# genometools/vstree

Measured on AMD Instinct MI355X. Metric: queries/sec (100 bp queries, vmatch -mum -l 20 semantics, 3 Gbp ESA index resident in HBM), higher is better.
Workload: dtype u8; 1 GPU; 3 Gbp synthetic DNA index, 10 M x 100 bp queries per GPU, -mum -l 20; index_bp=3000000000, queries_per_gpu=10000000, query_len=100, minlen=20, prefixlength=13, index_bytes_hbm=115012207262, reads_in_hbm=two bits per symbol, 32 bytes per read (vsa_pack_reads), parallelism=index replicated, queries sharded x1

## Files before the change

### vstree_amd/csrc/esa_search.hip

```cpp
#include "search_host.hpp"
#include <rocprim/rocprim.hpp>
#include <type_traits>

#include "search_complete.inc"
#include "search_query.inc"
#include "mum_workplan.inc"
#include "mem_workplan.inc"
#include "mum_filter.inc"
#include "candidate_sort.inc"
#include <atomic>


namespace
{


enum class Form
{
  Ref,
  Deep,
  Staged,
  Rows,
  Windows
};
// ... 370 lines not shown
        cand.as<vsa_match>(), ncand, lenbits, k1.as<uint64_t>(),
        i1.as<uint32_t>());
    VSA_HIP(hipGetLastError());
    if (sort_radix<uint32_t>(k1.as<uint64_t>(), i1.as<uint32_t>(), s, 0,
                             lenbits + dbbits, stream) ||
        mumfilter_tiles<true>(
            s, s.pairs(lenbits, GatheredRecord{cand.as<vsa_match>()}), carry,
            stream, mums, &c))
    {
      return -100;
    }
  }
  *nmums = c.nmums;
  *sumlength = c.sumlength;
  return 0;
}

struct RecordForm
{
  bool keeppairs;
  bool packed;
  unsigned int lenbits, dbbits;
  uint32_t packbits, valbits;
  size_t recsize;
};

int recordform(const vsa_index *index, const vsa_queries *queries, bool domum,
               bool domumcand, bool ordered, uint32_t forcebits,
               RecordForm *rf)
{
  const unsigned int need = bitsfor(queries->maxlength);
  rf->keeppairs = domum && domumcand && !ordered && forcebits != 0;
  rf->lenbits = rf->keeppairs ? forcebits : need;
  rf->dbbits = bitsfor(index->n);
  rf->packed = domum && (!domumcand || rf->keeppairs) &&
               rf->lenbits + rf->dbbits <= 64 && rf->lenbits >= need &&
               queries->maxlength < 0xFFFFu &&
               ((queries->nq + queries->seqoffset) >> 48) == 0;
  if (rf->keeppairs && !rf->packed)
  {
    VSA_ERROR("packed candidates: %u length bits do not fit this batch "
              "(longest query %lu, index %lu)", forcebits,
              (unsigned long) queries->maxlength, (unsigned long) index->n);
    return -2;
  }
  rf->packbits = rf->packed ? rf->lenbits : 0;
  const bool small = ((queries->nq << rf->lenbits) >> 32) == 0;
  rf->valbits = (rf->packed && !rf->keeppairs && small) ? rf->lenbits : 0;
  rf->recsize = rf->valbits != 0 ? 4 : (rf->packed ? 8 : sizeof(vsa_match));
  return 0;
}

int compact_into(const RecordForm &form, DevBuf &raw, DevBuf &rawkeys,
                 uint64_t cap, DevBuf &cursors, DevBuf &doff, DevBuf &out,
                 DevBuf &keys, uint64_t at, hipStream_t stream)
{
  auto launch = [&](auto rec) {
    using REC = decltype(rec);
    k_compact_shards<REC><<<VSA_CURSOR_SHARDS, VSA_BLOCK, 0, stream>>>(
        raw.as<REC>(), rawkeys.as<uint64_t>(), cap,
        cursors.as<unsigned long long>(), doff.as<uint64_t>(),
        out.as<REC>() + at, keys.as<uint64_t>() + at);
  };
  if (form.valbits != 0)
  {
    launch(uint32_t());
  } else if (form.packed)
  {
    launch(uint64_t());
  } else
  {
    launch(vsa_match());
  }
  VSA_HIP(hipGetLastError());
  return 0;
}

struct QueryRun
{
  const vsa_index *index;
  const vsa_queries *queries;
  hipStream_t stream;
  DevQueries qs;
  bool domum, domumcand, ordered;
  uint32_t searchlength;
  RecordForm rec;
  Timer tall, tsearch, tfirst;
  DevBuf base;
  const uint64_t *dbase = nullptr;
  uint32_t perquery = 0;
  uint64_t nitems = 0;
  bool reduce = false, memplan = false;
  Form form = Form::Ref;
  DevBuf wcount, wtemp, wplan, wlist, wfirste, wfmlen, wfmdb, wboffset;
  const uint64_t *nlistword = nullptr;
  DevBuf pcursor, pdoff, psummary, prawout, prawkeys;
  uint64_t pcap = 0;
  bool fromplan = false, planemit = false;
  uint64_t plansearches = 0;
  DevBuf cursor, doff, summary, blocksum, rtemp, rawout, rawkeys, out, keys;
  uint64_t shardcap = 0, needed = 0, nplan = 0, nfirst = 0, plannedwork = 0;
  uint64_t plannedlocates = 0;
  double searchms = 0;

  QueryRun(const vsa_index *ix, const vsa_queries *q, bool mum, bool cand,
           bool ord, uint32_t least)
      : index(ix), queries(q), stream(ix->stream), qs(devqueries(q)),
        domum(mum), domumcand(cand), ordered(ord), searchlength(least),
        tall(stream), tsearch(stream), tfirst(stream)
  {
  }
};

template <typename IDX>
int workitems(QueryRun &st)
{
  const uint64_t nqr = st.queries->nq, least = st.searchlength;
  if (st.qs.uniformlen != 0)
  {
    st.perquery = (st.qs.uniformlen >= least) ? st.qs.uniformlen - least + 1
                                              : 0;
    st.nitems = (uint64_t) st.perquery * nqr;
    return 0;
  }
  DevBuf btemp;
  auto items = rocprim::make_transform_iterator(
      rocprim::counting_iterator<uint64_t>(0),
      [len = st.qs.length, nqr, least] __device__(uint64_t q) -> uint64_t {
        if (q >= nqr)
        {
          return 0;
        }
        const uint64_t l = len[q];
        return l >= least ? l - least + 1 : 0;
      });
  if (st.base.alloc((nqr + 1) * 8))
  {
    return -100;
  }
  VSA_HIP(rocprim_run(btemp, [&](void *p, size_t &tb) {
    return rocprim::exclusive_scan(p, tb, items, st.base.as<uint64_t>(),
                                   (uint64_t) 0, (size_t) (nqr + 1),
                                   rocprim::plus<uint64_t>(), st.stream);
  }));
  st.dbase = st.base.as<uint64_t>();
  const Fetch f = {st.dbase + nqr, 8};
  return fetchwords(st.stream, &f, 1, &st.nitems) ? -100 : 0;
}

int decide(QueryRun &st)
{
  const vsa_index *index = st.index;
  const vsa_queries *queries = st.queries;
  const uint64_t maxoffsets =
      (queries->maxlength >= st.searchlength)
          ? queries->maxlength - st.searchlength + 1
          : 0;
  if (st.domum && queries->maxlength >= 255 && index->lcpquirk < 0)
  {
    uint8_t b = 0;
    if (index->n >= 2)
    {
      VSA_HIP(hipMemcpyAsync(&b, index->lcp + index->n - 1, 1,
                             hipMemcpyDeviceToHost, st.stream));
      VSA_HIP(hipStreamSynchronize(st.stream));
    }
    index->lcpquirk = (b == 255) ? 1 : 0;
  }
  const bool exhaustive = (index->tune & 2u) != 0;
  const bool planable = maxoffsets > 1 && maxoffsets < 0xFFFFu &&
                        queries->nq < 0xFFFFFFFFull && !exhaustive;
  st.reduce = st.domum && planable &&
              !(queries->maxlength >= 255 && index->lcpquirk != 0);
  st.memplan = !st.domum && planable && index->esa8 != nullptr &&
               st.searchlength >= index->D && st.searchlength <= 255;
  st.form = pickform(index, queries, st.qs,
                     st.reduce ? Stage::MumFirst : Stage::Bytes,
                     st.searchlength);
  if (queries->rows != nullptr && st.form < Form::Rows)
  {
    if (vsa_queries_bytes(queries, st.stream) != 0)
    {
      return -100;
    }
    st.qs = devqueries(queries);
  }
  return 0;
}

template <typename IDX>
int first_pass(QueryRun &st, const DevIndex<IDX> &ix, Form form,
               uint64_t *blockcount)
{
  st.tfirst.start();
  withform(form, [&](auto deep, auto pq, auto rows, auto windows) {
    k_mum_first<IDX, deep, pq, rows, windows>
        <<<gridfor(st.queries->nq), VSA_BLOCK, ldsbytes(form, st.qs),
           st.stream>>>(ix, st.qs, st.perquery, st.searchlength,
                        st.wcount.as<uint32_t>(), st.wfirste.as<uint32_t>(),
                        st.wfmlen.as<uint32_t>(), st.wfmdb.as<uint64_t>(),
                        blockcount);
  });
  st.tfirst.stop();
  VSA_HIP(hipGetLastError());
  return 0;
}

int alloc_first(QueryRun &st)
{
  const uint64_t nq = st.queries->nq;
  return st.wcount.alloc((nq + 1) * 4) || st.wfirste.alloc(nq * 4) ||
         st.wfmlen.alloc(nq * 4) || st.wfmdb.alloc(nq * 8) ||
         st.wplan.alloc(nq * sizeof(PlanRanges));
}

int plan_emit(QueryRun &st, uint32_t rounds, PlanEmit *em)
{
  const uint32_t nshards = VSA_CURSOR_SHARDS;
  const uint64_t nb = blocksfor(st.queries->nq),
                 pershard = (nb + nshards - 1) / nshards;
  st.pcap = pershard * VSA_BLOCK * rounds;
  if (st.pcursor.alloc((size_t) nshards * VSA_CURSOR_STRIDE * 8) ||
      st.pdoff.alloc(nshards * 8) || st.psummary.alloc(4 * 8) ||
      st.prawout.alloc(nshards * st.pcap * st.rec.recsize) ||
      st.prawkeys.alloc(nshards * st.pcap * 8))
  {
    return -100;
  }
  VSA_HIP(hipMemsetAsync(st.pcursor.p, 0,
                         (size_t) nshards * VSA_CURSOR_STRIDE * 8, st.stream));
  em->base = st.dbase;
  em->perquery = st.perquery;
  em->out = st.prawout.as<vsa_match>();
  em->outkey = st.prawkeys.as<uint64_t>();
  em->shardcap = st.pcap;
  em->shardmask = nshards - 1;
  em->cursors = st.pcursor.as<unsigned long long>();
  em->packbits = st.rec.packbits;
  em->valbits = st.rec.valbits;
  st.planemit = true;
  return 0;
}

hipError_t plan_summary(QueryRun &st)
{
  return shard_summary(st.pcursor.as<unsigned long long>(), VSA_CURSOR_SHARDS,
                       st.pdoff.as<uint64_t>(), st.psummary.as<uint64_t>(),
                       st.stream);
}

template <typename IDX>
int mem_plan(QueryRun &st, const DevIndex<IDX> &ix)
{
  const vsa_index *index = st.index;
  const uint64_t nq = st.queries->nq;
  if (index->repbits == nullptr || index->repleast != st.searchlength)
  {
    if (index->repbits == nullptr)
    {
      VSA_HIP(vsa_hip_malloc((void **) &index->repbits,
                             ((index->n + 1) / 32 + 4) * 4));
    }
    VSA_HIP(hipMemsetAsync(index->repbits, 0, ((index->n + 1) / 32 + 4) * 4,
                           st.stream));
    k_repeat_bits<IDX><<<vsa_grid(blocksfor((index->n + 16) / 16)),
                         VSA_BLOCK, 0, st.stream>>>(
        ix.lcp, ix.suf, index->n, st.searchlength, index->repbits);
    VSA_HIP(hipGetLastError());
    index->repleast = st.searchlength;
  }
  const Form first = pickform(index, st.queries, st.qs, Stage::MemFirst,
                              st.searchlength);
  PlanEmit em;
  if (alloc_first(st) || first_pass(st, ix, first, nullptr) ||
      plan_emit(st, VSA_PLAN_ROUNDS, &em))
  {
    return -100;
  }
  k_mem_plan<IDX><<<gridfor(nq), VSA_BLOCK, 0, st.stream>>>(
      ix, st.qs, st.perquery, st.searchlength, st.wfirste.as<uint32_t>(),
      st.wfmdb.as<uint64_t>(), index->repbits, st.wcount.as<uint32_t>(),
      st.wplan.as<PlanRanges>(), em);
  VSA_HIP(hipGetLastError());
  VSA_HIP(plan_summary(st));
  st.fromplan = true;
  st.plansearches = nq;
  return 0;
}

int dump_planfile(QueryRun &st, const char *pf)
{
  const uint64_t k = std::min<uint64_t>(st.queries->nq, 65536);
  std::vector<uint32_t> hc(k), hp(k * VSA_PLAN_RANGES);
  VSA_HIP(hipMemcpyAsync(hc.data(), st.wcount.p, k * 4,
                         hipMemcpyDeviceToHost, st.stream));
  VSA_HIP(hipMemcpyAsync(hp.data(), st.wplan.p, k * sizeof(PlanRanges),
                         hipMemcpyDeviceToHost, st.stream));
  VSA_HIP(hipStreamSynchronize(st.stream));
  if (FILE *f = fopen(pf, "wb"))
  {
    for (uint64_t q = 0; q < k; q++)
    {
      (void) fwrite(&hc[q], 4, 1, f);
      (void) fwrite(&hp[q * VSA_PLAN_RANGES], 4, VSA_PLAN_RANGES, f);
    }
    fclose(f);
  }
  return 0;
}

template <typename IDX>
int mum_plan(QueryRun &st, const DevIndex<IDX> &ix)
{
  const uint64_t nq = st.queries->nq;
  if (alloc_first(st) || st.wlist.alloc(nq * 4))
  {
    return -100;
  }
  VSA_HIP(hipMemsetAsync(st.wcount.as<uint32_t>() + nq, 0, 4, st.stream));
  const uint64_t nb = blocksfor(nq), nbr = vsa_grid_blocks(nb);
  DevBuf bcount;
  if (bcount.alloc((nbr + 1) * 8) || st.wboffset.alloc((nbr + 1) * 8))
  {
    return -100;
  }
  VSA_HIP(hipMemsetAsync(bcount.as<uint64_t>() + nb, 0, 8, st.stream));
  if (first_pass(st, ix, st.form, bcount.as<uint64_t>()))
  {
    return -100;
  }
  VSA_HIP(rocprim_run(st.wtemp, [&](void *p, size_t &tb) {
    return rocprim::exclusive_scan(p, tb, bcount.as<uint64_t>(),
                                   st.wboffset.as<uint64_t>(), (uint64_t) 0,
                                   (size_t) (nb + 1), rocprim::plus<uint64_t>(),
                                   st.stream);
  }));
  k_wanted_fill<<<vsa_grid(nb), VSA_BLOCK, 0, st.stream>>>(
      st.wcount.as<uint32_t>(), nq, 0u, st.wboffset.as<uint64_t>(),
      st.wlist.as<uint32_t>());
  VSA_HIP(hipGetLastError());
  st.nlistword = st.wboffset.as<uint64_t>() + nb;
  PlanEmit em = PlanEmit();
  if (st.form != Form::Ref && plan_emit(st, VSA_PLAN_ROUNDS - 1, &em))
  {
    return -100;
  }
  withform(st.form, [&](auto deep, auto, auto rows, auto) {
    k_mum_plan<IDX, deep, deep, rows><<<gridfor(nq), VSA_BLOCK, 0, st.stream>>>(
        ix, st.qs, st.wlist.as<uint32_t>(), st.nlistword, st.searchlength,
        st.wfirste.as<uint32_t>(), st.wcount.as<uint32_t>(),
        st.wplan.as<PlanRanges>(), em);
  });
  if (st.planemit)
  {
    VSA_HIP(plan_summary(st));
  }
  VSA_HIP(hipGetLastError());
  const char *pf = getenv("VSA_DEBUG_PLANFILE");
  if (pf != nullptr && dump_planfile(st, pf))
  {
    return -100;
  }
  st.fromplan = true;
  return 0;
}

bool tilequeue(const QueryRun &st)
{
  return st.fromplan && st.domum && (st.index->tune & 32u) == 0;
}

template <typename IDX>
int walkgrid(const QueryRun &st, uint32_t *grid)
{
  const vsa_index *index = st.index;
  if (index->walkgridasked != 0)
  {
    *grid = index->walkgridasked;
    return 0;
  }
  hipError_t e = hipSuccess;
  withform(st.form, [&](auto deep, auto, auto rows, auto) {
    uint32_t &kept = index->walkgrid[deep ? 1 : 0][rows ? 1 : 0];
    if (kept == 0)
    {
      int percu = 0, cus = 0;
      e = hipOccupancyMaxActiveBlocksPerMultiprocessor(
          &percu, k_mum_walk_tiles<IDX, deep, rows>, 256, 0);
      if (e == hipSuccess)
      {
        e = hipDeviceGetAttribute(&cus, hipDeviceAttributeMultiprocessorCount,
                                  index->device);
      }
      if (e == hipSuccess)
      {
        kept = (uint32_t) std::max(percu, 1) * (uint32_t) std::max(cus, 1);
      }
    }
    *grid = kept;
  });
  VSA_HIP(e);
  return 0;
}

template <typename IDX>
void launch_search(QueryRun &st, const DevIndex<IDX> &ix,
                   uint64_t nplanblocks, uint32_t regions)
{
  withform(st.form, [&](auto deep, auto, auto rows, auto) {
    auto tiles = [&]() {
      unsigned long long *cursors = st.cursor.as<unsigned long long>();
      k_mum_walk_tiles<IDX, deep, rows>
          <<<vsa_grid(nplanblocks), 256, 0, st.stream>>>(
              ix, st.qs, st.dbase, st.perquery, st.wplan.as<PlanRanges>(),
              st.wcount.as<uint32_t>(), st.wlist.as<uint32_t>(), st.nlistword,
              cursors + (size_t) VSA_CURSOR_SHARDS * VSA_CURSOR_STRIDE,
              st.searchlength, st.rawout.as<vsa_match>(),
              st.rawkeys.as<uint64_t>(), st.shardcap, regions - 1, cursors,
              st.rec.packbits, st.rec.valbits,
              st.blocksum.as<PlannedWork>(), st.index->walkshift);
    };
    auto planned = [&](auto mum) {
      k_query_search_planned<IDX, 256, deep, rows, mum>
          <<<vsa_grid(nplanblocks), 256, 0, st.stream>>>(
              ix, st.qs, st.dbase, st.perquery, st.wplan.as<PlanRanges>(),
              st.wcount.as<uint32_t>(), st.searchlength,
              st.rawout.as<vsa_match>(), st.rawkeys.as<uint64_t>(),
              st.shardcap, VSA_CURSOR_SHARDS - 1,
              st.cursor.as<unsigned long long>(), st.rec.packbits,
              st.rec.valbits, st.blocksum.as<PlannedWork>(),
              st.index->walkshift);
    };
    auto unplanned = [&](auto mum) {
      k_query_search<IDX, mum, deep, 256>
          <<<vsa_grid((st.nitems + 255) / 256), 256, 0, st.stream>>>(
              ix, st.qs, st.dbase, st.perquery, st.nitems, st.searchlength,
              st.rawout.as<vsa_match>(), st.rawkeys.as<uint64_t>(),
              st.shardcap, VSA_CURSOR_SHARDS - 1,
              st.cursor.as<unsigned long long>(), st.rec.packbits,
              st.rec.valbits);
    };
    if (tilequeue(st))
    {
      tiles();
    } else if (st.fromplan && st.domum)
    {
      planned(std::true_type());
    } else if (st.fromplan)
    {
      if constexpr (deep && !rows)
      {
        planned(std::false_type());
      }
    } else if (st.nitems > 0 && st.domum)
    {
      unplanned(std::true_type());
    } else if (st.nitems > 0)
    {
      unplanned(std::false_type());
    }
  });
}

template <typename IDX>
int search(QueryRun &st, const DevIndex<IDX> &ix)
{
  const uint32_t nshards = VSA_CURSOR_SHARDS;
  const uint64_t perblock = 256 * (st.domum ? VSA_WALK_READS : 1);
  uint64_t nplanblocks = (st.queries->nq + perblock - 1) / perblock;
  uint64_t persum = 1;
  size_t rbytes = 0;
  if (tilequeue(st))
  {
    uint32_t grid = 0;
    if (walkgrid<IDX>(st, &grid))
    {
      return -100;
    }
    nplanblocks = grid;
    persum = 4;
  }
  const uint64_t nsums = persum * nplanblocks;
  if (st.fromplan)
  {
    if (st.blocksum.alloc((persum * vsa_grid_blocks(nplanblocks) + 1) *
                          sizeof(PlannedWork)))
    {
      return -100;
    }
    VSA_HIP(rocprim::reduce(nullptr, rbytes, st.blocksum.as<PlannedWork>(),
                            (PlannedWork *) nullptr, PlannedWork{0, 0},
                            (size_t) nsums, PlannedWorkPlus(), st.stream));
    if (st.rtemp.alloc(rbytes))
    {
      return -100;
    }
  }
  const size_t cursorbytes = (size_t) (nshards + 1) * VSA_CURSOR_STRIDE * 8;
  if (st.cursor.alloc(cursorbytes) || st.doff.alloc(nshards * 8) ||
      st.summary.alloc(6 * 8))
  {
    return -100;
  }
  st.shardcap =
      std::max<uint64_t>((st.queries->nq * 2 / nshards) * 5 / 4 + 64, 256);
  uint64_t maxshard = 0;
  uint32_t regions = nshards;
  for (int attempt = 0; attempt < 2; attempt++)
  {
    if (st.rawout.alloc(regions * st.shardcap * st.rec.recsize) ||
        st.rawkeys.alloc(regions * st.shardcap * 8))
    {
      return -100;
    }
    VSA_HIP(hipMemsetAsync(st.cursor.p, 0, cursorbytes, st.stream));
    st.tsearch.start();
    launch_search(st, ix, nplanblocks, regions);
    st.tsearch.stop();
    VSA_HIP(hipGetLastError());
    if (st.fromplan)
    {
      VSA_HIP(rocprim::reduce(
          st.rtemp.p, rbytes, st.blocksum.as<PlannedWork>(),
          reinterpret_cast<PlannedWork *>(st.summary.as<uint64_t>() + 4),
          PlannedWork{0, 0}, (size_t) nsums, PlannedWorkPlus(), st.stream));
    }
    const uint64_t *sm = st.summary.as<uint64_t>();
    VSA_HIP(shard_summary(st.cursor.as<unsigned long long>(), nshards,
                          st.doff.as<uint64_t>(), st.summary.as<uint64_t>(),
                          st.stream));
    const Fetch f[8] = {{sm, 8}, {sm + 1, 8}, {sm + 2, 8}, {sm + 3, 8},
                        {sm + 4, 8}, {st.planemit ? st.psummary.p : sm, 8},
                        {st.nlistword != nullptr ? st.nlistword : sm, 8},
                        {sm + 5, 8}};
    uint64_t got[8];
    if (fetchwords(st.stream, f, 8, got))
    {
      return -100;
    }
    if (st.nlistword != nullptr)
    {
      st.nfirst = got[6] >> 32;
      st.plansearches = 2 * (got[6] & 0xFFFFFFFFull);
    }
    st.nplan = st.planemit ? got[5] : 0;
    st.needed = got[0];
    maxshard = got[1];
    st.plannedlocates = st.fromplan ? got[4] : 0;
    st.plannedwork = st.fromplan ? got[7] : 0;
    st.searchms += st.tsearch.ms();
    if (maxshard <= st.shardcap)
    {
      return 0;
    }
    st.shardcap = maxshard;
    if (tilequeue(st))
    {
      regions = 1;
      st.shardcap = st.needed;
    }
  }
  VSA_ERROR("match buffer overflow: %llu > %llu",
            (unsigned long long) maxshard, (unsigned long long) st.shardcap);
  return -5;
}

int compact(QueryRun &st)
{
  const uint64_t total = st.needed + st.nplan + st.nfirst;
  if (total == 0)
  {
    return 0;
  }
  if (st.out.alloc(total * st.rec.recsize) || st.keys.alloc(total * 8) ||
      (st.nplan > 0 &&
       compact_into(st.rec, st.prawout, st.prawkeys, st.pcap, st.pcursor,
                    st.pdoff, st.out, st.keys, st.needed, st.stream)) ||
      (st.needed > 0 &&
       compact_into(st.rec, st.rawout, st.rawkeys, st.shardcap, st.cursor,
                    st.doff, st.out, st.keys, 0, st.stream)))
  {
    return -100;
  }
  if (st.nfirst > 0)
  {
    k_append_first<<<gridfor(st.queries->nq), VSA_BLOCK, 0, st.stream>>>(
        st.wfmlen.as<uint32_t>(), st.wfmdb.as<uint64_t>(),
        st.wboffset.as<uint64_t>(), st.queries->nq, st.perquery, st.dbase,
        st.qs.seqoffset, st.needed + st.nplan, st.out.as<vsa_match>(),
        st.keys.as<uint64_t>(), st.rec.packbits, st.rec.valbits);
    VSA_HIP(hipGetLastError());
  }
  st.needed = total;
  return 0;
}

#define VSA_CS_MINPAIRS (1u << 14)

std::atomic<uint64_t> g_cs_runs{0}, g_cs_overflows{0}, g_cs_longruns{0},
    g_cs_shift{0}, g_cs_buckets{0};

bool feedsbuckets(const QueryRun &st)
{
  const uint64_t total = st.needed + st.nplan + st.nfirst;
  const uint32_t tune = st.index->tune;
  if (!(st.domum && !st.domumcand && st.rec.packed && (tune & 4u) == 0 &&
        total > 0 && (total >= VSA_CS_MINPAIRS || (tune & 8u) != 0) &&
        cs_geometry(st.index->n, total, st.rec.lenbits, st.rec.dbbits)
                .nbuckets <= VSA_CS_MAXBUCKETS))
  {
    return false;
  }
  if ((tune & 8u) == 0 && st.index->cs_skip > 0)
  {
    st.index->cs_skip--;
    return false;
  }
  return true;
}

template <typename VAL>
int mumfilter_buckets(QueryRun &st, DevBuf &mums, MumCounts *c)
{
  const RecordForm &rec = st.rec;
  const uint64_t total = st.needed + st.nplan + st.nfirst;
  CsSources src = CsSources();
  if (st.needed > 0)
  {
    src.reg[0] = {st.rawout.p, st.rawkeys.as<uint64_t>(),
                  st.cursor.as<unsigned long long>(), st.shardcap, st.needed};
  }
  if (st.nplan > 0)
  {
    src.reg[1] = {st.prawout.p, st.prawkeys.as<uint64_t>(),
                  st.pcursor.as<unsigned long long>(), st.pcap, st.nplan};
  }
  if (st.nfirst > 0)
  {
    src.first = {st.wfmlen.as<uint32_t>(), st.wfmdb.as<uint64_t>(),
                 st.queries->nq, st.qs.seqoffset, rec.packbits, rec.valbits};
  }
  CsGeometry g;
  if (mums.alloc(total * sizeof(vsa_match)))
  {
    return -100;
  }
  const PairRecord<VAL> pr = {rec.lenbits, rec.valbits,
                              sizeof(VAL) == 4 ? st.qs.seqoffset : 0};
  uint64_t got[3];
  if (candidate_bucketfilter<VAL>(src, total, st.index->n, rec.lenbits,
                                  rec.dbbits, 0, pr, st.stream,
                                  mums.as<vsa_match>(), got, &g))
  {
    return -100;
  }
  g_cs_runs++;
  g_cs_shift = g.shift;
  g_cs_buckets = g.nbuckets;
  c->nmums = got[0];
  c->sumlength = got[1];
  c->flags = got[2];
  return 0;
}

int finish(QueryRun &st, vsa_result *res, uint64_t *mumsum)
{
  const RecordForm &rec = st.rec;
  bool allbits = false;
  if (feedsbuckets(st))
  {
    DevBuf mums;
    MumCounts c;
    if (rec.valbits != 0 ? mumfilter_buckets<uint32_t>(st, mums, &c)
                         : mumfilter_buckets<uint64_t>(st, mums, &c))
    {
      return -100;
    }
    if (c.flags == 0)
    {
      st.index->cs_penalty = 0;
      res->stats.candidates = st.needed + st.nplan + st.nfirst;
      res->count = c.nmums;
      res->matches = (vsa_match *) mums.release();
      *mumsum = c.sumlength;
      return 0;
    }
    if ((c.flags & VSA_CS_OVERFLOW) != 0)
    {
// ... 497 lines not shown
```

### vstree_amd/csrc/mum_workplan.inc

```



#define VSA_PLAN_RANGES 4
#define VSA_PLAN_ROUNDS 6
#define VSA_PLAN_UNKNOWN 0xFFFFFFFFu

#ifndef VSA_PLAN_WAVES
#define VSA_PLAN_WAVES 1
#endif
#ifndef VSA_FIRST_WAVES
#define VSA_FIRST_WAVES 1
#endif
struct PlanRanges
{
  uint32_t r[VSA_PLAN_RANGES];
};

__device__ __forceinline__ void plan_add(PlanRanges &pr, uint32_t &nr,
                                         uint32_t first, uint32_t last)
{
  if (first > last)
  {
    return;
  }
// ... 548 lines not shown
{
  uint32_t q[VSA_WALK_ASIDE], r[VSA_WALK_ASIDE];
};

__device__ __forceinline__ void vsa_wave_lds_fence()
{
  __builtin_amdgcn_fence(__ATOMIC_RELEASE, "wavefront");
  __builtin_amdgcn_wave_barrier();
  __builtin_amdgcn_fence(__ATOMIC_ACQUIRE, "wavefront");
}

__device__ __forceinline__ uint32_t vsa_rank_in(uint64_t mask)
{
  return __builtin_amdgcn_mbcnt_hi(
      (uint32_t) (mask >> 32), __builtin_amdgcn_mbcnt_lo((uint32_t) mask, 0u));
}

__device__ __forceinline__ void vsa_plan_chunk(const PlanRanges &p, uint32_t r,
                                               uint32_t cshift,
                                               uint32_t &first, uint32_t &off)
{
  const uint32_t chunk = 1u << cshift;
#pragma unroll
  for (int k = 0; k < VSA_PLAN_RANGES; k++)
  {
    const uint32_t rf = p.r[k] & 0xFFFFu, len = p.r[k] >> 16,
                   nchunks = (len + chunk - 1) >> cshift;
    if (r < nchunks)
    {
      const uint32_t at = r << cshift, n = len - at < chunk ? len - at : chunk;
      first = rf + at;
      off = first + n - 1;
      r = 0xFFFFFFFFu;
    } else if (r != 0xFFFFFFFFu)
    {
      r -= nchunks;
    }
  }
}

template <typename IDX, bool DEEP = true, bool ROWS = false>
__global__ void __launch_bounds__(256, VSA_WALK_WAVES)
k_mum_walk_tiles(const DevIndex<IDX> ix, const DevQueries qs,
                 const uint64_t *__restrict__ base, uint32_t perquery,
                 const PlanRanges *__restrict__ plan,
                 const uint32_t *__restrict__ plancount,
                 const uint32_t *__restrict__ list,
                 const uint64_t *__restrict__ nlistword,
                 unsigned long long *__restrict__ tilecounter,
                 uint32_t searchlength, vsa_match *__restrict__ out,
                 uint64_t *__restrict__ outkey, uint64_t shardcap,
                 uint32_t shardmask, unsigned long long *__restrict__ cursors,
                 uint32_t packbits, uint32_t valbits,
                 PlannedWork *__restrict__ blocksum, uint32_t chunkshift)
{
  __shared__ WalkTile tiles[4];
  __shared__ WalkAside asides[ROWS ? 4 : 1];
  const uint32_t lane = threadIdx.x & 63u, wave = threadIdx.x >> 6;
  WalkTile &tile = tiles[wave];
  WalkAside &aside = asides[ROWS ? wave : 0];
  const uint64_t nlist = *nlistword & 0xFFFFFFFFull;
  const uint32_t shard = vsa_bid() & shardmask;
  uint32_t head = 0, tail = 0, naside = 0;
  bool exhausted = false;
  bool active = false;
  uint32_t off = 0, first = 0, q = 0, qlen = qs.uniformlen;
  uint32_t locates = 0, offsets = 0;
  const uint8_t *qstart = qs.symbols;
  for (;;)
  {
    uint64_t freemask = __ballot(!active);
    while (freemask != 0 && !(ROWS && naside >= 64))
    {
      if (head == tail)
      {
        if (exhausted)
        {
          break;
        }
        unsigned long long mine = 0;
        if (lane == 0)
        {
          mine = atomicAdd(tilecounter, 1ull);
        }
        const uint64_t t0 =
            ((uint64_t) __builtin_amdgcn_readfirstlane((uint32_t) (mine >> 32))
             << 32) |
            __builtin_amdgcn_readfirstlane((uint32_t) mine);
        if (t0 * 64 >= nlist)
        {
          exhausted = true;
          break;
        }
        const uint64_t t = t0 * 64 + lane;
        uint32_t tq = 0, nch = 0;
        PlanRanges p;
#pragma unroll
        for (int g = 0; g < VSA_PLAN_RANGES; g++)
        {
          p.r[g] = 0;
        }
        if (t < nlist)
        {
          tq = list[t];
          const uint32_t c = plancount[tq];
          p = plan[tq];
          offsets += c;
// ... 88 lines not shown
            arq.valid = 0;
            src.row = qs.rows;
            src.bytes = nullptr;
            src.pos = src.m = 0;
            if (mine)
            {
              aq = aside.q[a0 + lane];
              afirst = aside.r[a0 + lane] & 0xFFFFu;
              aoff = aside.r[a0 + lane] >> 16;
              (void) vsa_row_of(qs, aq, qs.uniformlen, arq, src);
            }
            locates += vsa_walk_chunk<IDX, true, false>(
                ix, qs, mine, src, nullptr, qlen, afirst, aoff, aq, base,
                perquery, searchlength, out, outkey, shardcap, shard, cursors,
                packbits, valbits);
          }
          vsa_wave_lds_fence();
          naside = 0;
          q = first = off = 0;
          continue;
        }
      }
      break;
    }
    if constexpr (DEEP && ROWS)
    {
      RowQuery rq;
      QSrc src;
      rq.row = qs.rows + (uint64_t) q * qs.roww;
      rq.valid = qlen;
      src.row = rq.row;
      src.bytes = nullptr;
      src.pos = 0;
      src.m = (int32_t) qlen;
      vsa_walk_step<IDX, true, true>(ix, qs, active, src, &rq, qlen, first,
                                     off, q, base, perquery, searchlength, out,
                                     outkey, shardcap, shard, cursors, packbits,
                                     valbits, locates);
    } else
    {
      vsa_walk_step<IDX, DEEP, false>(ix, qs, active, qstart, nullptr, qlen,
                                      first, off, q, base, perquery,
                                      searchlength, out, outkey, shardcap,
                                      shard, cursors, packbits, valbits,
                                      locates);
    }
  }
  uint64_t sum = locates | ((uint64_t) offsets << 32);
#pragma unroll
  for (int d = 32; d >= 1; d >>= 1)
  {
    sum += vsa_shfl64(sum, (int) lane ^ d);
  }
  if (lane == 0)
  {
    blocksum[vsa_bid() * 4 + wave] =
        PlannedWork{sum & 0xFFFFFFFFull, sum >> 32};
  }
}

template <typename IDX, bool DEEP, bool PQ = false, bool ROWS = false,
          bool WINDOWS = false>
__global__ void __launch_bounds__(VSA_BLOCK, VSA_FIRST_WAVES)
k_mum_first(const DevIndex<IDX> ix, const DevQueries qs, uint32_t perquery,
            uint32_t searchlength, uint32_t *__restrict__ count,
            uint32_t *__restrict__ firste, uint32_t *__restrict__ fmlen,
            uint64_t *__restrict__ fmdb,
            uint64_t *__restrict__ blockcount = nullptr)
{
  extern __shared__ uint32_t stagedqueries[];
  __shared__ uint32_t wantwaves[VSA_BLOCK / 64], candwaves[VSA_BLOCK / 64];
  const uint64_t q = vsa_bid() * VSA_BLOCK + threadIdx.x;
  uint32_t qlen = qs.uniformlen, perq = perquery;
  const uint8_t *qptr = qs.symbols;
  uint32_t maxlcp = 0;
  uint64_t witness = 0;
  bool have = false, fast = false;
  DeepHit hit;

  if (!ROWS && q < qs.nq)
  {
    if (qs.dense)
    {
      qptr = qs.symbols + q * qs.uniformlen;
    } else
    {
      qptr = qs.symbols + qs.start[q];
      qlen = (uint32_t) qs.length[q];
      perq = (qlen >= searchlength) ? qlen - searchlength + 1 : 0;
    }
  }
  const bool active = q < qs.nq && perq > 0;
  if constexpr (DEEP && ROWS && WINDOWS)
  {
    RowQuery rq;
    QSrc src;
    bool flagged = false;
    rq.row = qs.rows;
    rq.valid = 0;
    src.row = qs.rows;
    src.bytes = nullptr;
    src.pos = src.m = 0;
    if (q < qs.nq)
    {
      flagged = vsa_row_of(qs, q, qlen, rq, src);
    }
    int st = vsa_locate_deep<3, true>(ix, active && !flagged, src, qlen,
                                      maxlcp, witness, hit, 0xFFFFFFFFu,
                                      0x100u, &rq, 0);
    if (active && flagged)
    {
      st = VSA_LOC_SLOW;
    }
    if (st == VSA_LOC_SLOW)
    {
      have = vsa_locate_reference(ix, src, qlen, maxlcp, witness);
    } else
    {
      have = st == VSA_LOC_FOUND;
      fast = have && maxlcp < 255;
    }
// ... 27 lines not shown
    if constexpr (PQ)
    {
      PackedQuery pq;
      vsa_pq_stage<VSA_BLOCK>(qs, vsa_bid() * VSA_BLOCK, qlen,
                              stagedqueries, pq);
      st = vsa_locate_deep<3, true>(ix, active, qptr, qlen, maxlcp,
                                           witness, hit, 0xFFFFFFFFu, 0x100u,
                                           &pq);
    } else
    {
      st = vsa_locate_deep<3>(ix, active, qptr, qlen, maxlcp, witness, hit);
    }
    if (st == VSA_LOC_SLOW)
    {
      have = vsa_locate_reference(ix, qptr, qlen, maxlcp, witness);
    } else
    {
      have = st == VSA_LOC_FOUND;
      fast = have && maxlcp < 255;
    }
  } else
  {
    if (active)
    {
      have = vsa_locate_reference(ix, qptr, qlen, maxlcp, witness);
    }
  }
  uint32_t len = 0, wanted = 0;
  if (q < qs.nq)
  {
    uint64_t db = 0;
    if (active && have && maxlcp >= searchlength)
    {
      bool unique;
      if (fast)
      {
        const uint32_t lcpw = (uint32_t) (hit.ew >> 32) & 0xFFu;
        unique = (witness == 0 || lcpw < maxlcp) &&
                 (witness + 1 > ix.n - 1 || hit.lcpnext < maxlcp);
        db = vsa_entrystart(ix, hit.ew, witness);
      } else
      {
        unique = vsa_mum_candidate<IDX, DEEP>(ix, maxlcp, witness);
        db = vsa_sufstart<IDX, DEEP>(ix, witness);
      }
      len = unique ? maxlcp : 0;
    }
    wanted = !active ? 0 : ((have && maxlcp >= qlen) ? 0 : perq);
    fmlen[q] = len;
    fmdb[q] = db;
    firste[q] = (active && have) ? maxlcp : VSA_PLAN_UNKNOWN;
    count[q] = wanted;
  }
  if (blockcount != nullptr)
  {
    const uint64_t wmask = __ballot(wanted > 0), cmask = __ballot(len != 0);
    if ((threadIdx.x & 63) == 0)
    {
      wantwaves[threadIdx.x >> 6] = (uint32_t) __popcll(wmask);
      candwaves[threadIdx.x >> 6] = (uint32_t) __popcll(cmask);
    }
    __syncthreads();
    if (threadIdx.x == 0)
    {
      uint64_t t = 0, f = 0;
#pragma unroll
      for (int w = 0; w < VSA_BLOCK / 64; w++)
      {
        t += wantwaves[w];
        f += candwaves[w];
      }
      blockcount[vsa_bid()] = t | (f << 32);
    }
  }
}

__global__ void __launch_bounds__(VSA_BLOCK)
k_append_first(const uint32_t *__restrict__ fmlen,
               const uint64_t *__restrict__ fmdb,
               const uint64_t *__restrict__ blockoffset, uint64_t nq,
               uint32_t perquery, const uint64_t *__restrict__ qbase,
               uint64_t seqoffset, uint64_t base,
               vsa_match *__restrict__ out, uint64_t *__restrict__ outkey,
               uint32_t packbits, uint32_t valbits)
{
  __shared__ uint32_t waves[VSA_BLOCK / 64];
  const uint64_t q = vsa_bid() * VSA_BLOCK + threadIdx.x;
  const bool have = q < nq && fmlen[q] != 0;
  const uint64_t mask = __ballot(have);
  const uint32_t lane = threadIdx.x & 63, wave = threadIdx.x >> 6;
  if (lane == 0)
  {
    waves[wave] = (uint32_t) __popcll(mask);
  }
  __syncthreads();
  if (!have)
  {
    return;
  }
  uint64_t slot = (blockoffset[vsa_bid()] >> 32) +
                  (uint32_t) __popcll(mask & ((1ull << lane) - 1));
#pragma unroll
  for (uint32_t w = 0; w < VSA_BLOCK / 64; w++)
  {
    slot += (w < wave) ? waves[w] : 0u;
  }
  if (packbits != 0)
  {
    outkey[base + slot] =
        (fmdb[q] << packbits) | (((1ull << packbits) - 1) - fmlen[q]);
    if (valbits != 0)
    {
      reinterpret_cast<uint32_t *>(out)[base + slot] =
          (uint32_t) (q << valbits);
    } else
    {
      reinterpret_cast<uint64_t *>(out)[base + slot] =
          (q + seqoffset) << 16;
    }
  } else
  {
    vsa_match m;
    m.length = fmlen[q];
    m.dbstart = fmdb[q];
    m.queryseq = q + seqoffset;
    m.querystart = 0;
    out[base + slot] = m;
    outkey[base + slot] = (qbase != nullptr) ? qbase[q] : q * perquery;
  }
}

struct NonZeroToU32
{
  __device__ uint32_t operator()(uint32_t v) const
  {
    return v != 0 ? 1u : 0u;
  }
};

__global__ void __launch_bounds__(VSA_BLOCK)
k_wanted_fill(const uint32_t *__restrict__ count, uint64_t nq,
              uint32_t threshold, const uint64_t *__restrict__ blockoffset,
              uint32_t *__restrict__ list)
{
  __shared__ uint32_t waves[VSA_BLOCK / 64];
  const uint64_t q = vsa_bid() * VSA_BLOCK + threadIdx.x;
  const bool want = q < nq && count[q] > threshold;
  const uint64_t mask = __ballot(want);
  const uint32_t lane = threadIdx.x & 63, wave = threadIdx.x >> 6;
  if (lane == 0)
  {
    waves[wave] = (uint32_t) __popcll(mask);
  }
  __syncthreads();
  if (want)
  {
    uint32_t at = (uint32_t) blockoffset[vsa_bid()] +
                  (uint32_t) __popcll(mask & ((1ull << lane) - 1));
#pragma unroll
    for (uint32_t w = 0; w < VSA_BLOCK / 64; w++)
    {
      at += (w < wave) ? waves[w] : 0u;
    }
    list[at] = (uint32_t) q;
  }
}

struct PlanWanted
{
  const uint32_t *count;
  uint32_t threshold;
  __device__ bool operator()(uint32_t q) const
  {
    return count[q] > threshold;
  }
};
```

### vstree_amd/csrc/search_common.hip

```cpp
#include "search_host.hpp"
#include <rocprim/rocprim.hpp>

namespace
{

#define VSA_FETCH_MAX 8
struct FetchList
{
  const void *src[VSA_FETCH_MAX];
  uint32_t bytes[VSA_FETCH_MAX];
  int count;
};

__global__ void k_fetch_words(const FetchList list, uint64_t *__restrict__ page)
{
  const int i = threadIdx.x;
  if (i < list.count)
  {
    uint64_t v = 0;
    const uint8_t *p = (const uint8_t *) list.src[i];
    if (list.bytes[i] == 8)
    {
      v = *(const uint64_t *) p;
    } else
// ... 97 lines not shown
  if (k != 0)
  {
    const uint4 *src = reinterpret_cast<const uint4 *>(in + t);
    uint4 *dst = reinterpret_cast<uint4 *>(out + s);
    const uint4 lo = src[0], hi = src[1];
    dst[0] = lo;
    dst[1] = hi;
  }
  if (t == count - 1)
  {
    *nkept = (uint64_t) s + k;
  }
}

struct MatchLength
{
  __device__ uint64_t operator()(const vsa_match &m) const
  {
    return m.length;
  }
};

__global__ void __launch_bounds__(VSA_BLOCK)
k_iota_u32(uint32_t *__restrict__ out, uint64_t n)
{
  const uint64_t t = vsa_bid() * VSA_BLOCK + threadIdx.x;
  if (t < n)
  {
    out[t] = (uint32_t) t;
  }
}

__global__ void __launch_bounds__(VSA_BLOCK)
k_gather_matches(const vsa_match *__restrict__ in,
                 const uint32_t *__restrict__ order, uint64_t n,
                 vsa_match *__restrict__ out)
{
  const uint64_t t = vsa_bid() * VSA_BLOCK + threadIdx.x;
  if (t < n)
  {
    const uint4 *src = reinterpret_cast<const uint4 *>(in + order[t]);
    uint4 *dst = reinterpret_cast<uint4 *>(out + t);
    const uint4 lo = src[0], hi = src[1];
    dst[0] = lo;
    dst[1] = hi;
  }
}

__global__ void __launch_bounds__(1024)
k_shard_summary(const unsigned long long *__restrict__ cursors,
                uint32_t nshards, uint64_t *__restrict__ offsets,
                const uint32_t *__restrict__ extra_a,
                const uint32_t *__restrict__ extra_b,
                uint64_t *__restrict__ summary)
{
  __shared__ uint64_t sums[1024], maxs[1024];
  const uint32_t per = (nshards + 1023) / 1024, t = threadIdx.x;
  uint64_t mine = 0, mx = 0;
  for (uint32_t k = 0; k < per; k++)
  {
    const uint32_t sh = t * per + k;
    if (sh < nshards)
    {
      const uint64_t c = cursors[(uint64_t) sh * VSA_CURSOR_STRIDE];
      mine += c;
      mx = c > mx ? c : mx;
    }
  }
  sums[t] = mine;
  maxs[t] = mx;
  __syncthreads();
  for (uint32_t d = 1; d < 1024; d <<= 1)
  {
    const uint64_t a = t >= d ? sums[t - d] : 0,
                   b = t >= d ? maxs[t - d] : 0;
    __syncthreads();
    sums[t] += a;
    maxs[t] = b > maxs[t] ? b : maxs[t];
    __syncthreads();
  }
  uint64_t run = sums[t] - mine;
  for (uint32_t k = 0; k < per; k++)
  {
    const uint32_t sh = t * per + k;
    if (sh < nshards)
    {
      offsets[sh] = run;
      run += cursors[(uint64_t) sh * VSA_CURSOR_STRIDE];
    }
  }
  if (t == 1023)
  {
    summary[0] = sums[t];
    summary[1] = maxs[t];
    summary[2] = extra_a != nullptr ? *extra_a : 0;
    summary[3] = extra_b != nullptr ? *extra_b : 0;
  }
}

}

hipError_t shard_summary(const unsigned long long *cursors, uint32_t nshards,
                         uint64_t *offsets, uint64_t *summary,
                         hipStream_t stream)
{
  k_shard_summary<<<1, 1024, 0, stream>>>(cursors, nshards, offsets, nullptr,
                                          nullptr, summary);
  return hipGetLastError();
}

int compact_matches(const vsa_match *in, const uint8_t *keep,
                           uint64_t count, vsa_match *out, uint64_t *nkept,
                           hipStream_t stream)
{
  DevBuf slots, temp;
  auto keepit = rocprim::make_transform_iterator(keep, KeepToU32());

  if (slots.alloc(count * 4))
  {
    return -100;
  }
  VSA_HIP(rocprim_run(temp, [&](void *p, size_t &tb) {
    return rocprim::exclusive_scan(p, tb, keepit, slots.as<uint32_t>(),
                                   (uint32_t) 0, (size_t) count,
                                   rocprim::plus<uint32_t>(), stream);
  }));
  k_scatter_kept<<<gridfor(count), VSA_BLOCK, 0, stream>>>(
      in, keep, slots.as<uint32_t>(), count, out, nkept);
  VSA_HIP(hipGetLastError());
  return 0;
}

int exclusive_sum(uint64_t *counts, uint64_t *offsets, uint64_t n,
                  hipStream_t stream, uint64_t *total)
{
  DevBuf temp;
  VSA_HIP(rocprim_run(temp, [&](void *p, size_t &tb) {
    return rocprim::exclusive_scan(p, tb, counts, offsets, (uint64_t) 0,
                                   (size_t) (n + 1),
                                   rocprim::plus<uint64_t>(), stream);
  }));
  const Fetch f = {offsets + n, 8};
  return fetchwords(stream, &f, 1, total);
}

int sumlengths(const vsa_match *matches, uint64_t n, hipStream_t stream,
               uint64_t *result)
{
  *result = 0;
  if (n == 0)
  {
    return 0;
  }
  DevBuf out, temp;
  auto in = rocprim::make_transform_iterator(matches, MatchLength());
  if (out.alloc(sizeof(uint64_t)) != 0)
  {
    return -100;
  }
  VSA_HIP(rocprim_run(temp, [&](void *p, size_t &tb) {
// ... 70 lines not shown
```

### vstree_amd/csrc/search_host.hpp

```cpp
#ifndef VSA_SEARCH_HOST_HPP
#define VSA_SEARCH_HOST_HPP
#include <cstring>
#include <algorithm>
#include "esa_device.hpp"

#define VSA_BLOCK 256
#define VSA_CURSOR_STRIDE 8
#define VSA_CURSOR_SHARDS 2048
#define VSA_HIDDEN __attribute__((visibility("hidden")))

struct DevBuf
{
  void *p = nullptr;
  ~DevBuf()
  {
    vsa_dev_free(p);
  }
  void free()
  {
    vsa_dev_free(p);
    p = nullptr;
  }
  int alloc(size_t bytes)
  {
// ... 148 lines not shown
                         hipStream_t stream);

VSA_HIDDEN int sortpairs(uint64_t *keys_in, uint64_t *keys_out,
                         uint32_t *vals_in, uint32_t *vals_out, uint64_t n,
                         unsigned int endbit, hipStream_t stream);

VSA_HIDDEN vsa_result *newresult(int device);

struct ResultGuard
{
  vsa_result *r;
  ~ResultGuard()
  {
    if (r != nullptr)
    {
      vsa_result_free(r);
    }
  }
};

inline int enter(int device)
{
  if (vsa_set_device(device) != 0)
  {
    return -100;
  }
  vsa_dev_set_stream(nullptr);
  return 0;
}

inline int upload_queryview(uint64_t nq, const uint64_t **qstart,
                            const uint64_t **qlen, uint64_t **d_qstart,
                            uint64_t **d_qlen, const char *who)
{
  const size_t bytes = (size_t) nq * 8;
  if (*qstart != nullptr && bytes > 0 &&
      (vsa_hip_malloc((void **) d_qstart, bytes) != hipSuccess ||
       vsa_hip_malloc((void **) d_qlen, bytes) != hipSuccess ||
       hipMemcpy(*d_qstart, *qstart, bytes, hipMemcpyHostToDevice) !=
           hipSuccess ||
       hipMemcpy(*d_qlen, *qlen, bytes, hipMemcpyHostToDevice) != hipSuccess))
  {
    VSA_ERROR("%s: upload of the query Multiseq failed", who);
    return -100;
  }
  *qstart = *d_qstart;
  *qlen = *d_qlen;
  return 0;
}

VSA_HIDDEN hipError_t shard_summary(const unsigned long long *cursors,
                                    uint32_t nshards, uint64_t *offsets,
                                    uint64_t *summary, hipStream_t stream);

struct U32ToU64
{
  __device__ uint64_t operator()(uint32_t v) const
  {
    return v;
  }
};

#endif
```

Before: 4.168 billion queries/s.

## Fold wanted-list fill and work sums into kernels via atomics, merge cursor buffers

The first-pass kernel now claims its block's list offset with an atomicAdd and writes the wanted-query list directly. This removes the separate exclusive scan and k_wanted_fill launch. The walk kernel accumulates planned-work totals with global atomics instead of per-wave block sums plus a rocprim reduce. The plan and search cursors share one allocation that is zeroed once, and both shard summaries run in a single two-block launch. Together these cut kernel launches and memsets per batch. In exchange, list order now depends on atomic ordering, which is nondeterministic, and atomics add contention.

```diff
diff --git a/vstree_amd/csrc/esa_search.hip b/vstree_amd/csrc/esa_search.hip
--- a/vstree_amd/csrc/esa_search.hip
+++ b/vstree_amd/csrc/esa_search.hip
@@ -446,15 +446,15 @@
 }
 
 int compact_into(const RecordForm &form, DevBuf &raw, DevBuf &rawkeys,
-                 uint64_t cap, DevBuf &cursors, DevBuf &doff, DevBuf &out,
-                 DevBuf &keys, uint64_t at, hipStream_t stream)
+                 uint64_t cap, const unsigned long long *cursors, DevBuf &doff,
+                 DevBuf &out, DevBuf &keys, uint64_t at, hipStream_t stream)
 {
   auto launch = [&](auto rec) {
     using REC = decltype(rec);
     k_compact_shards<REC><<<VSA_CURSOR_SHARDS, VSA_BLOCK, 0, stream>>>(
         raw.as<REC>(), rawkeys.as<uint64_t>(), cap,
-        cursors.as<unsigned long long>(), doff.as<uint64_t>(),
-        out.as<REC>() + at, keys.as<uint64_t>() + at);
+        cursors, doff.as<uint64_t>(), out.as<REC>() + at,
+        keys.as<uint64_t>() + at);
   };
   if (form.valbits != 0)
   {
@@ -486,13 +486,15 @@
   uint64_t nitems = 0;
   bool reduce = false, memplan = false;
   Form form = Form::Ref;
-  DevBuf wcount, wtemp, wplan, wlist, wfirste, wfmlen, wfmdb, wboffset;
-  const uint64_t *nlistword = nullptr;
-  DevBuf pcursor, pdoff, psummary, prawout, prawkeys;
+  DevBuf wcount, wplan, wlist, wfirste, wfmlen, wfmdb, wboffset;
+  uint64_t *nlistword = nullptr;
+  unsigned long long *pcursor = nullptr;
+  DevBuf pdoff, psummary, prawout, prawkeys;
   uint64_t pcap = 0;
   bool fromplan = false, planemit = false;
   uint64_t plansearches = 0;
   DevBuf cursor, doff, summary, blocksum, rtemp, rawout, rawkeys, out, keys;
+  bool cursorsfresh = false;
   uint64_t shardcap = 0, needed = 0, nplan = 0, nfirst = 0, plannedwork = 0;
   uint64_t plannedlocates = 0;
   double searchms = 0;
@@ -583,8 +585,7 @@
 }
 
 template <typename IDX>
-int first_pass(QueryRun &st, const DevIndex<IDX> &ix, Form form,
-               uint64_t *blockcount)
+int first_pass(QueryRun &st, const DevIndex<IDX> &ix, Form form, bool list)
 {
   st.tfirst.start();
   withform(form, [&](auto deep, auto pq, auto rows, auto windows) {
@@ -593,7 +594,10 @@
            st.stream>>>(ix, st.qs, st.perquery, st.searchlength,
                         st.wcount.as<uint32_t>(), st.wfirste.as<uint32_t>(),
                         st.wfmlen.as<uint32_t>(), st.wfmdb.as<uint64_t>(),
-                        blockcount);
+                        list ? reinterpret_cast<unsigned long long *>(
+                                   st.nlistword)
+                             : nullptr,
+                        st.wboffset.as<uint64_t>(), st.wlist.as<uint32_t>());
   });
   st.tfirst.stop();
   VSA_HIP(hipGetLastError());
@@ -608,39 +612,57 @@
          st.wplan.alloc(nq * sizeof(PlanRanges));
 }
 
+#define VSA_CURSOR_LINES (2 * VSA_CURSOR_SHARDS + 2)
+#define VSA_SEARCH_LINES (VSA_CURSOR_SHARDS + 2)
+
+int alloc_cursors(QueryRun &st)
+{
+  if (st.cursor.p != nullptr)
+  {
+    return 0;
+  }
+  const size_t bytes = (size_t) VSA_CURSOR_LINES * VSA_CURSOR_STRIDE * 8;
+  if (st.cursor.alloc(bytes))
+  {
+    return -100;
+  }
+  VSA_HIP(hipMemsetAsync(st.cursor.p, 0, bytes, st.stream));
+  st.cursorsfresh = true;
+  st.pcursor = st.cursor.as<unsigned long long>() +
+               (size_t) VSA_SEARCH_LINES * VSA_CURSOR_STRIDE;
+  return 0;
+}
+
+unsigned long long *worksums(QueryRun &st)
+{
+  return st.cursor.as<unsigned long long>() +
+         (size_t) (VSA_CURSOR_SHARDS + 1) * VSA_CURSOR_STRIDE;
+}
+
 int plan_emit(QueryRun &st, uint32_t rounds, PlanEmit *em)
 {
   const uint32_t nshards = VSA_CURSOR_SHARDS;
   const uint64_t nb = blocksfor(st.queries->nq),
                  pershard = (nb + nshards - 1) / nshards;
   st.pcap = pershard * VSA_BLOCK * rounds;
-  if (st.pcursor.alloc((size_t) nshards * VSA_CURSOR_STRIDE * 8) ||
-      st.pdoff.alloc(nshards * 8) || st.psummary.alloc(4 * 8) ||
+  if (alloc_cursors(st) || st.pdoff.alloc(nshards * 8) ||
+      st.psummary.alloc(4 * 8) ||
       st.prawout.alloc(nshards * st.pcap * st.rec.recsize) ||
       st.prawkeys.alloc(nshards * st.pcap * 8))
   {
     return -100;
   }
-  VSA_HIP(hipMemsetAsync(st.pcursor.p, 0,
-                         (size_t) nshards * VSA_CURSOR_STRIDE * 8, st.stream));
   em->base = st.dbase;
   em->perquery = st.perquery;
   em->out = st.prawout.as<vsa_match>();
   em->outkey = st.prawkeys.as<uint64_t>();
   em->shardcap = st.pcap;
   em->shardmask = nshards - 1;
-  em->cursors = st.pcursor.as<unsigned long long>();
+  em->cursors = st.pcursor;
   em->packbits = st.rec.packbits;
   em->valbits = st.rec.valbits;
   st.planemit = true;
   return 0;
-}
-
-hipError_t plan_summary(QueryRun &st)
-{
-  return shard_summary(st.pcursor.as<unsigned long long>(), VSA_CURSOR_SHARDS,
-                       st.pdoff.as<uint64_t>(), st.psummary.as<uint64_t>(),
-                       st.stream);
 }
 
 template <typename IDX>
@@ -666,7 +688,7 @@
   const Form first = pickform(index, st.queries, st.qs, Stage::MemFirst,
                               st.searchlength);
   PlanEmit em;
-  if (alloc_first(st) || first_pass(st, ix, first, nullptr) ||
+  if (alloc_first(st) || first_pass(st, ix, first, false) ||
       plan_emit(st, VSA_PLAN_ROUNDS, &em))
   {
     return -100;
@@ -676,7 +698,6 @@
       st.wfmdb.as<uint64_t>(), index->repbits, st.wcount.as<uint32_t>(),
       st.wplan.as<PlanRanges>(), em);
   VSA_HIP(hipGetLastError());
-  VSA_HIP(plan_summary(st));
   st.fromplan = true;
   st.plansearches = nq;
   return 0;
@@ -712,30 +733,15 @@
     return -100;
   }
   VSA_HIP(hipMemsetAsync(st.wcount.as<uint32_t>() + nq, 0, 4, st.stream));
-  const uint64_t nb = blocksfor(nq), nbr = vsa_grid_blocks(nb);
-  DevBuf bcount;
-  if (bcount.alloc((nbr + 1) * 8) || st.wboffset.alloc((nbr + 1) * 8))
-  {
-    return -100;
-  }
-  VSA_HIP(hipMemsetAsync(bcount.as<uint64_t>() + nb, 0, 8, st.stream));
-  if (first_pass(st, ix, st.form, bcount.as<uint64_t>()))
-  {
-    return -100;
-  }
-  VSA_HIP(rocprim_run(st.wtemp, [&](void *p, size_t &tb) {
-    return rocprim::exclusive_scan(p, tb, bcount.as<uint64_t>(),
-                                   st.wboffset.as<uint64_t>(), (uint64_t) 0,
-                                   (size_t) (nb + 1), rocprim::plus<uint64_t>(),
-                                   st.stream);
-  }));
-  k_wanted_fill<<<vsa_grid(nb), VSA_BLOCK, 0, st.stream>>>(
-      st.wcount.as<uint32_t>(), nq, 0u, st.wboffset.as<uint64_t>(),
-      st.wlist.as<uint32_t>());
-  VSA_HIP(hipGetLastError());
-  st.nlistword = st.wboffset.as<uint64_t>() + nb;
+  const uint64_t nbr = vsa_grid_blocks(blocksfor(nq));
   PlanEmit em = PlanEmit();
-  if (st.form != Form::Ref && plan_emit(st, VSA_PLAN_ROUNDS - 1, &em))
+  if (st.wboffset.alloc(nbr * 8) || alloc_cursors(st) ||
+      (st.form != Form::Ref && plan_emit(st, VSA_PLAN_ROUNDS - 1, &em)))
+  {
+    return -100;
+  }
+  st.nlistword = reinterpret_cast<uint64_t *>(worksums(st) + 2);
+  if (first_pass(st, ix, st.form, true))
   {
     return -100;
   }
@@ -745,10 +751,6 @@
         st.wfirste.as<uint32_t>(), st.wcount.as<uint32_t>(),
         st.wplan.as<PlanRanges>(), em);
   });
-  if (st.planemit)
-  {
-    VSA_HIP(plan_summary(st));
-  }
   VSA_HIP(hipGetLastError());
   const char *pf = getenv("VSA_DEBUG_PLANFILE");
   if (pf != nullptr && dump_planfile(st, pf))
@@ -811,8 +813,8 @@
               cursors + (size_t) VSA_CURSOR_SHARDS * VSA_CURSOR_STRIDE,
               st.searchlength, st.rawout.as<vsa_match>(),
               st.rawkeys.as<uint64_t>(), st.shardcap, regions - 1, cursors,
-              st.rec.packbits, st.rec.valbits,
-              st.blocksum.as<PlannedWork>(), st.index->walkshift);
+              st.rec.packbits, st.rec.valbits, worksums(st),
+              st.index->walkshift);
     };
     auto planned = [&](auto mum) {
       k_query_search_planned<IDX, 256, deep, rows, mum>
@@ -862,9 +864,9 @@
   const uint32_t nshards = VSA_CURSOR_SHARDS;
   const uint64_t perblock = 256 * (st.domum ? VSA_WALK_READS : 1);
   uint64_t nplanblocks = (st.queries->nq + perblock - 1) / perblock;
-  uint64_t persum = 1;
   size_t rbytes = 0;
-  if (tilequeue(st))
+  const bool tiles = tilequeue(st);
+  if (tiles)
   {
     uint32_t grid = 0;
     if (walkgrid<IDX>(st, &grid))
@@ -872,12 +874,11 @@
       return -100;
     }
     nplanblocks = grid;
-    persum = 4;
-  }
-  const uint64_t nsums = persum * nplanblocks;
-  if (st.fromplan)
-  {
-    if (st.blocksum.alloc((persum * vsa_grid_blocks(nplanblocks) + 1) *
+  }
+  const uint64_t nsums = nplanblocks;
+  if (st.fromplan && !tiles)
+  {
+    if (st.blocksum.alloc((vsa_grid_blocks(nplanblocks) + 1) *
                           sizeof(PlannedWork)))
     {
       return -100;
@@ -890,8 +891,9 @@
       return -100;
     }
   }
-  const size_t cursorbytes = (size_t) (nshards + 1) * VSA_CURSOR_STRIDE * 8;
-  if (st.cursor.alloc(cursorbytes) || st.doff.alloc(nshards * 8) ||
+  const size_t cursorbytes =
+      (size_t) (nshards + 1) * VSA_CURSOR_STRIDE * 8 + 2 * 8;
+  if (alloc_cursors(st) || st.doff.alloc(nshards * 8) ||
       st.summary.alloc(6 * 8))
   {
     return -100;
@@ -907,12 +909,16 @@
     {
       return -100;
     }
-    VSA_HIP(hipMemsetAsync(st.cursor.p, 0, cursorbytes, st.stream));
+    if (!st.cursorsfresh)
+    {
+      VSA_HIP(hipMemsetAsync(st.cursor.p, 0, cursorbytes, st.stream));
+    }
+    st.cursorsfresh = false;
     st.tsearch.start();
     launch_search(st, ix, nplanblocks, regions);
     st.tsearch.stop();
     VSA_HIP(hipGetLastError());
-    if (st.fromplan)
+    if (st.fromplan && !tiles)
     {
       VSA_HIP(rocprim::reduce(
           st.rtemp.p, rbytes, st.blocksum.as<PlannedWork>(),
@@ -920,13 +926,17 @@
           PlannedWork{0, 0}, (size_t) nsums, PlannedWorkPlus(), st.stream));
     }
     const uint64_t *sm = st.summary.as<uint64_t>();
-    VSA_HIP(shard_summary(st.cursor.as<unsigned long long>(), nshards,
-                          st.doff.as<uint64_t>(), st.summary.as<uint64_t>(),
-                          st.stream));
+    const unsigned long long *ws = worksums(st);
+    VSA_HIP(shard_summary_pair(
+        st.cursor.as<unsigned long long>(), st.doff.as<uint64_t>(),
+        st.summary.as<uint64_t>(), st.planemit ? st.pcursor : nullptr,
+        st.pdoff.as<uint64_t>(), st.psummary.as<uint64_t>(), nshards,
+        st.stream));
     const Fetch f[8] = {{sm, 8}, {sm + 1, 8}, {sm + 2, 8}, {sm + 3, 8},
-                        {sm + 4, 8}, {st.planemit ? st.psummary.p : sm, 8},
+                        {tiles ? (const void *) ws : sm + 4, 8},
+                        {st.planemit ? st.psummary.p : sm, 8},
                         {st.nlistword != nullptr ? st.nlistword : sm, 8},
-                        {sm + 5, 8}};
+                        {tiles ? (const void *) (ws + 1) : sm + 5, 8}};
     uint64_t got[8];
     if (fetchwords(st.stream, f, 8, got))
     {
@@ -971,8 +981,8 @@
        compact_into(st.rec, st.prawout, st.prawkeys, st.pcap, st.pcursor,
                     st.pdoff, st.out, st.keys, st.needed, st.stream)) ||
       (st.needed > 0 &&
-       compact_into(st.rec, st.rawout, st.rawkeys, st.shardcap, st.cursor,
-                    st.doff, st.out, st.keys, 0, st.stream)))
+       compact_into(st.rec, st.rawout, st.rawkeys, st.shardcap,
+                    st.cursor.as<unsigned long long>(), st.doff, st.out, st.keys, 0, st.stream)))
   {
     return -100;
   }
@@ -1027,7 +1037,7 @@
   if (st.nplan > 0)
   {
     src.reg[1] = {st.prawout.p, st.prawkeys.as<uint64_t>(),
-                  st.pcursor.as<unsigned long long>(), st.pcap, st.nplan};
+                  st.pcursor, st.pcap, st.nplan};
   }
   if (st.nfirst > 0)
   {
diff --git a/vstree_amd/csrc/mum_workplan.inc b/vstree_amd/csrc/mum_workplan.inc
--- a/vstree_amd/csrc/mum_workplan.inc
+++ b/vstree_amd/csrc/mum_workplan.inc
@@ -624,7 +624,8 @@
                  uint64_t *__restrict__ outkey, uint64_t shardcap,
                  uint32_t shardmask, unsigned long long *__restrict__ cursors,
                  uint32_t packbits, uint32_t valbits,
-                 PlannedWork *__restrict__ blocksum, uint32_t chunkshift)
+                 unsigned long long *__restrict__ worksum,
+                 uint32_t chunkshift)
 {
   __shared__ WalkTile tiles[4];
   __shared__ WalkAside asides[ROWS ? 4 : 1];
@@ -819,10 +820,9 @@
   {
     sum += vsa_shfl64(sum, (int) lane ^ d);
   }
-  if (lane == 0)
-  {
-    blocksum[vsa_bid() * 4 + wave] =
-        PlannedWork{sum & 0xFFFFFFFFull, sum >> 32};
+  if (lane < 2)
+  {
+    atomicAdd(worksum + lane, lane == 0 ? sum & 0xFFFFFFFFull : sum >> 32);
   }
 }
 
@@ -833,7 +833,9 @@
             uint32_t searchlength, uint32_t *__restrict__ count,
             uint32_t *__restrict__ firste, uint32_t *__restrict__ fmlen,
             uint64_t *__restrict__ fmdb,
-            uint64_t *__restrict__ blockcount = nullptr)
+            unsigned long long *__restrict__ listword = nullptr,
+            uint64_t *__restrict__ blockoffset = nullptr,
+            uint32_t *__restrict__ list = nullptr)
 {
   extern __shared__ uint32_t stagedqueries[];
   __shared__ uint32_t wantwaves[VSA_BLOCK / 64], candwaves[VSA_BLOCK / 64];
@@ -967,13 +969,14 @@
     firste[q] = (active && have) ? maxlcp : VSA_PLAN_UNKNOWN;
     count[q] = wanted;
   }
-  if (blockcount != nullptr)
+  if (listword != nullptr)
   {
     const uint64_t wmask = __ballot(wanted > 0), cmask = __ballot(len != 0);
-    if ((threadIdx.x & 63) == 0)
-    {
-      wantwaves[threadIdx.x >> 6] = (uint32_t) __popcll(wmask);
-      candwaves[threadIdx.x >> 6] = (uint32_t) __popcll(cmask);
+    const uint32_t lane = threadIdx.x & 63, wave = threadIdx.x >> 6;
+    if (lane == 0)
+    {
+      wantwaves[wave] = (uint32_t) __popcll(wmask);
+      candwaves[wave] = (uint32_t) __popcll(cmask);
     }
     __syncthreads();
     if (threadIdx.x == 0)
@@ -985,7 +988,21 @@
         t += wantwaves[w];
         f += candwaves[w];
       }
-      blockcount[vsa_bid()] = t | (f << 32);
+      const uint64_t start = atomicAdd(listword, t | (f << 32));
+      blockoffset[vsa_bid()] = start;
+      candwaves[0] = (uint32_t) start;
+    }
+    __syncthreads();
+    if (wanted > 0)
+    {
+      uint32_t at = candwaves[0] +
+                    (uint32_t) __popcll(wmask & ((1ull << lane) - 1));
+#pragma unroll
+      for (uint32_t w = 0; w < VSA_BLOCK / 64; w++)
+      {
+        at += (w < wave) ? wantwaves[w] : 0u;
+      }
+      list[at] = (uint32_t) q;
     }
   }
 }
@@ -1052,41 +1069,3 @@
     return v != 0 ? 1u : 0u;
   }
 };
-
-__global__ void __launch_bounds__(VSA_BLOCK)
-k_wanted_fill(const uint32_t *__restrict__ count, uint64_t nq,
-              uint32_t threshold, const uint64_t *__restrict__ blockoffset,
-              uint32_t *__restrict__ list)
-{
-  __shared__ uint32_t waves[VSA_BLOCK / 64];
-  const uint64_t q = vsa_bid() * VSA_BLOCK + threadIdx.x;
-  const bool want = q < nq && count[q] > threshold;
-  const uint64_t mask = __ballot(want);
-  const uint32_t lane = threadIdx.x & 63, wave = threadIdx.x >> 6;
-  if (lane == 0)
-  {
-    waves[wave] = (uint32_t) __popcll(mask);
-  }
-  __syncthreads();
-  if (want)
-  {
-    uint32_t at = (uint32_t) blockoffset[vsa_bid()] +
-                  (uint32_t) __popcll(mask & ((1ull << lane) - 1));
-#pragma unroll
-    for (uint32_t w = 0; w < VSA_BLOCK / 64; w++)
-    {
-      at += (w < wave) ? waves[w] : 0u;
-    }
-    list[at] = (uint32_t) q;
-  }
-}
-
-struct PlanWanted
-{
-  const uint32_t *count;
-  uint32_t threshold;
-  __device__ bool operator()(uint32_t q) const
-  {
-    return count[q] > threshold;
-  }
-};
diff --git a/vstree_amd/csrc/search_common.hip b/vstree_amd/csrc/search_common.hip
--- a/vstree_amd/csrc/search_common.hip
+++ b/vstree_amd/csrc/search_common.hip
@@ -173,9 +173,19 @@
                 uint32_t nshards, uint64_t *__restrict__ offsets,
                 const uint32_t *__restrict__ extra_a,
                 const uint32_t *__restrict__ extra_b,
-                uint64_t *__restrict__ summary)
+                uint64_t *__restrict__ summary,
+                const unsigned long long *__restrict__ cursors2 = nullptr,
+                uint64_t *__restrict__ offsets2 = nullptr,
+                uint64_t *__restrict__ summary2 = nullptr)
 {
   __shared__ uint64_t sums[1024], maxs[1024];
+  if (blockIdx.x == 1)
+  {
+    cursors = cursors2;
+    offsets = offsets2;
+    summary = summary2;
+    extra_a = extra_b = nullptr;
+  }
   const uint32_t per = (nshards + 1023) / 1024, t = threadIdx.x;
   uint64_t mine = 0, mx = 0;
   for (uint32_t k = 0; k < per; k++)
@@ -227,6 +237,18 @@
 {
   k_shard_summary<<<1, 1024, 0, stream>>>(cursors, nshards, offsets, nullptr,
                                           nullptr, summary);
+  return hipGetLastError();
+}
+
+hipError_t shard_summary_pair(const unsigned long long *cursors,
+                              uint64_t *offsets, uint64_t *summary,
+                              const unsigned long long *cursors2,
+                              uint64_t *offsets2, uint64_t *summary2,
+                              uint32_t nshards, hipStream_t stream)
+{
+  k_shard_summary<<<cursors2 != nullptr ? 2 : 1, 1024, 0, stream>>>(
+      cursors, nshards, offsets, nullptr, nullptr, summary, cursors2, offsets2,
+      summary2);
   return hipGetLastError();
 }
 
diff --git a/vstree_amd/csrc/search_host.hpp b/vstree_amd/csrc/search_host.hpp
--- a/vstree_amd/csrc/search_host.hpp
+++ b/vstree_amd/csrc/search_host.hpp
@@ -224,6 +224,12 @@
 VSA_HIDDEN hipError_t shard_summary(const unsigned long long *cursors,
                                     uint32_t nshards, uint64_t *offsets,
                                     uint64_t *summary, hipStream_t stream);
+VSA_HIDDEN hipError_t shard_summary_pair(const unsigned long long *cursors,
+                                         uint64_t *offsets, uint64_t *summary,
+                                         const unsigned long long *cursors2,
+                                         uint64_t *offsets2,
+                                         uint64_t *summary2, uint32_t nshards,
+                                         hipStream_t stream);
 
 struct U32ToU64
 {
```

New measurement: 4.123 billion queries/s. 0.989x the previous value.
